# stgl/scarplet

Measured on AMD Instinct MI355X. Metric: Mpixel·template/s (DEM pixels × ages × orientations / s), higher is better.
Workload: dtype f32

## Files before the change

scarplet_amd/csrc/sc_api.hip:

```cpp
#include "sc_internal.h"
#include <stdarg.h>
#include <stdio.h>
#include <string.h>
#include <stdlib.h>
#include <math.h>
#include <algorithm>

int sc_fail(sc_ctx* ctx, int code, const char* fmt, ...) {
    char buf[1024];
    va_list ap;
    va_start(ap, fmt);
    vsnprintf(buf, sizeof(buf), fmt, ap);
    va_end(ap);
    if (ctx) ctx->err = buf;
    return code;
}

int sc_ensure(sc_ctx* ctx, DevBuf& b, size_t bytes) {
    if (bytes <= b.cap && b.p) return SC_OK;
    if (b.p) {
        SC_HIP(ctx, hipFree(b.p));
        b.p = nullptr;
        b.cap = 0;
    }
// ... 27 lines not shown
    size_t s = 0;
    for (DevBuf* b : arr) s += b->cap;
    for (auto& w : c->windows) s += (size_t)w.h * w.wd * 13;
    return s;
}

int sc_lds_attr(sc_ctx* ctx, const void* kernel, size_t bytes) {
    auto it = ctx->lds_attr.find(kernel);
    if (it != ctx->lds_attr.end() && it->second >= bytes) return SC_OK;
    SC_HIP(ctx, hipFuncSetAttribute(kernel, hipFuncAttributeMaxDynamicSharedMemorySize,
                                    (int)bytes));
    ctx->lds_attr[kernel] = bytes;
    return SC_OK;
}

void sc_prof_begin(sc_ctx* ctx, int kernel) {
    ctx->prof_cur = -1;
    ctx->prof_kernel = kernel;
    const long long b = ctx->k_brackets[kernel]++;
    if (!ctx->prof) return;
    uint32_t h = (uint32_t)b * 2654435761u;
    h ^= h >> 15;
    h *= 2246822519u;
    h ^= h >> 13;
    if (ctx->prof > 1 && h % (uint32_t)ctx->prof) return;
    std::pair<hipEvent_t, hipEvent_t> ev;
    if (!ctx->ev_pool.empty()) {
        ev = ctx->ev_pool.back();
        ctx->ev_pool.pop_back();
    } else {
        if (hipEventCreate(&ev.first) != hipSuccess) return;
        if (hipEventCreate(&ev.second) != hipSuccess) return;
    }
    (void)hipEventRecord(ev.first, ctx->stream);
    ctx->prof_cur = kernel;
    ctx->prof_ev0 = ev.first;
    ctx->prof_ev1 = ev.second;
}

void sc_prof_end(sc_ctx* ctx, int n) {
    ctx->k_launches[ctx->prof_kernel] += n;
    if (ctx->prof_cur < 0) return;
    (void)hipEventRecord(ctx->prof_ev1, ctx->stream);
    ctx->pending.push_back({ctx->prof_cur, {ctx->prof_ev0, ctx->prof_ev1}});
    ctx->pending_n.push_back(n);
    ctx->prof_cur = -1;
}

void sc_prof_collect(sc_ctx* ctx) {
    for (size_t i = 0; i < ctx->pending.size(); ++i) {
        auto& p = ctx->pending[i];
        float ms = 0.f;
        if (hipEventElapsedTime(&ms, p.second.first, p.second.second) == hipSuccess) {
            ctx->k_ms[p.first] += ms;
            ctx->k_sampled[p.first] += ctx->pending_n[i];
        }
        ctx->ev_pool.push_back(p.second);
    }
// ... 6 lines not shown
extern "C" int sc_device_count(void) {
    int n = 0;
    if (hipGetDeviceCount(&n) != hipSuccess) return 0;
    return n;
}

extern "C" int sc_create(int device, sc_ctx** out) {
    if (!out) return SC_ERR_INVALID;
    *out = nullptr;
    int n = 0;
    if (hipGetDeviceCount(&n) != hipSuccess || n <= 0) return SC_ERR_HIP;
    if (device < 0 || device >= n) return SC_ERR_INVALID;
    if (hipSetDevice(device) != hipSuccess) return SC_ERR_HIP;
    sc_ctx* c = new sc_ctx();
    c->device = device;
    if (hipStreamCreateWithFlags(&c->stream, hipStreamNonBlocking) != hipSuccess) {
        delete c;
        return SC_ERR_HIP;
    }
    *out = c;
    return SC_OK;
}

extern "C" int sc_set_option(sc_ctx* ctx, const char* name, double value) {
    if (!ctx || !name) return SC_ERR_INVALID;
    if (!strcmp(name, "kappa")) {
        if (!(value >= 0.0)) return sc_fail(ctx, SC_ERR_INVALID, "kappa must be >= 0");
        ctx->kappa = (float)value;
    } else if (!strcmp(name, "variant")) {
        ctx->variant = (int)value;
    } else if (!strcmp(name, "batch")) {
// ... 12 lines not shown
        ctx->batch_templ = (int)value;
    } else if (!strcmp(name, "split_i1")) {
        if (!(value >= 0.0 && value <= 64.0)) return sc_fail(ctx, SC_ERR_INVALID, "split_i1 must be 0 .. 64");
        ctx->split_i1 = (int)value;
    } else if (!strcmp(name, "split_fill")) {
        if (!(value >= 0.0)) return sc_fail(ctx, SC_ERR_INVALID, "split_fill must be >= 0");
        ctx->split_fill = (long long)value;
    } else if (!strcmp(name, "sib")) {
        ctx->sib = (int)value;
    } else if (!strcmp(name, "spectra_mb")) {
        if (!(value >= 0.0)) return sc_fail(ctx, SC_ERR_INVALID, "spectra_mb must be >= 0");
        ctx->spec_mb = value;
        fft_spectra_forget(ctx);
    } else if (!strcmp(name, "fuse_fwd")) {
        ctx->fuse_fwd = value != 0.0;
    } else if (!strcmp(name, "y_gb")) {
        if (!(value >= 0.0)) return sc_fail(ctx, SC_ERR_INVALID, "y_gb must be >= 0");
        ctx->y_gb = value;
    } else if (!strcmp(name, "fit_chunk")) {
        if (!(value >= 0.0 && std::isfinite(value))) return sc_fail(ctx, SC_ERR_INVALID, "fit_chunk must be >= 0 and finite");
        ctx->fit_chunk = value >= 0x1p62 ? (1ll << 62) : (long long)value;
    } else if (!strcmp(name, "channel_terms")) {
        if (!(value == 0.0 || value == 1.0)) return sc_fail(ctx, SC_ERR_INVALID, "channel_terms must be 0 or 1");
        ctx->channel_terms = (int)value;
    } else {
        return sc_fail(ctx, SC_ERR_INVALID, "unknown option '%s'", name);
    }
    return SC_OK;
}

extern "C" int sc_clear_windows(sc_ctx* ctx) {
    if (!ctx) return SC_ERR_INVALID;
    (void)hipStreamSynchronize(ctx->stream);
    for (auto& w : ctx->windows) {
        if (!w.pooled) {
            if (w.w) (void)hipFree(w.w);
            if (w.w64) (void)hipFree(w.w64);
            if (w.m) (void)hipFree(w.m);
        }
        if (w.mask_lim) (void)hipFree(w.mask_lim);
        if (w.mask_err) (void)hipFree(w.mask_err);
    }
    ctx->windows.clear();
    for (void* p : ctx->window_pools) (void)hipFree(p);
    ctx->window_pools.clear();
    return SC_OK;
}

extern "C" void sc_destroy(sc_ctx* c) {
    if (!c) return;
    (void)hipSetDevice(c->device);
    (void)hipStreamSynchronize(c->stream);
    sc_comm_destroy(c);
    sc_prof_collect(c);
    for (auto& e : c->ev_pool) {
        (void)hipEventDestroy(e.first);
        (void)hipEventDestroy(e.second);
    }
    sc_clear_windows(c);
    DevBuf* arr[] = {&c->z, &c->xaxis, &c->yaxis, &c->A, &c->B, &c->C, &c->curv,
                     &c->best_snr, &c->best_amp, &c->best_id, &c->map_amp,
                     &c->map_snr, &c->templ, &c->sums, &c->wl1, &c->norms, &c->norm_part, &c->win_w, &c->win_m,
                     &c->tw_y, &c->tw_x, &c->blk, &c->cblk, &c->uc, &c->uc2, &c->vh, &c->wh, &c->mh,
                     &c->yw, &c->ym, &c->tiles, &c->halo_z, &c->halo_stage, &c->res, &c->sib_buf, &c->dwin, &c->spans, &c->res_stats, &c->digest, &c->split_s, &c->split_a, &c->split_i,
                     &c->near, &c->near_ev, &c->score, &c->score_w, &c->score_abc, &c->st_slot, &c->st_work, &c->st_pairs, &c->st_patch, &c->st_spans, &c->snap, &c->xch, &c->xch_cnt,
                     &c->tr_planes, &c->tr_thin, &c->tr_par, &c->tr_lab, &c->tr_cnt, &c->tr_bsum, &c->tr_tot, &c->tr_sort, &c->tr_hist, &c->tr_rbsum, &c->tr_seg,
                     &c->pf_z, &c->pf_cells, &c->pf_dir, &c->pf_ages, &c->pf_tab, &c->pf_rows, &c->pf_sse, &c->pf_shift, &c->pf_wt, &c->pf_ftab, &c->pf_terms,
                     &c->sg_z, &c->sg_ages, &c->sg_tab, &c->sg_cells, &c->sg_dir, &c->sg_cseg, &c->sg_start, &c->sg_blk, &c->sg_label, &c->sg_prof, &c->sg_int,
                     &c->sg_scal, &c->sg_age, &c->sg_list, &c->sg_part, &c->sg_tot, &c->sg_tsse, &c->sg_cnt, &c->sg_rows, &c->sg_out, &c->sg_sse, &c->sg_shift, &c->sg_ftab, &c->sg_width, &c->sg_fine, &c->sq_wt, &c->sq_state, &c->sq_hist, &c->sq_a,
                     &c->bs_blk, &c->bs_sblk, &c->bs_terms, &c->bs_index, &c->bs_a, &c->bs_hist, &c->bs_rows, &c->cb_rows, &c->cb_mb,
                     &c->st_win, &c->st_wstart, &c->st_spp, &c->st_rows, &c->st_sse, &c->cw_shift,
                     &c->sb_win, &c->sb_wstart, &c->sb_wblk, &c->sb_bhi, &c->sb_rows, &c->sb_hist,
                     &c->sf_work, &c->sf_cells, &c->sf_cube, &c->sf_rows};
    for (DevBuf* b : arr) buf_free(*b);
    for (int k = 0; k < 4; ++k) buf_free(c->cmp[k]);
    for (int k = 0; k < 4; ++k) buf_free(c->cmp_in[k]);
    for (int k = 0; k < 4; ++k) buf_free(c->fill[k]);
    (void)hipStreamDestroy(c->stream);
    delete c;
}

extern "C" const char* sc_last_error(sc_ctx* ctx) {
    return ctx ? ctx->err.c_str() : "null context";
}

extern "C" size_t sc_device_bytes(sc_ctx* ctx) { return ctx ? sc_total_bytes(ctx) : 0; }

static int set_dem_body(sc_ctx* ctx, int ly, int lx, int gy0, int gx0, int ny,
                        int nx, int cy0, int cy1, int cx0, int cx1, double dx,
                        double dy, int wrap, const double* xaxis,
                        const double* yaxis);

// ... 373 lines not shown
    for (int j = 0; j < n; ++j) {
        if (t[j].kind == SC_KIND_WINDOW) ctx->h_wslot[j] = t[j].window;
        ctx->h_mix[3 * (size_t)j] = t[j].cc;
        ctx->h_mix[3 * (size_t)j + 1] = t[j].sc2;
        ctx->h_mix[3 * (size_t)j + 2] = t[j].ss;
        ctx->templ_windows = ctx->templ_windows || t[j].kind == SC_KIND_WINDOW;
    }
}

int sc_load_templates(sc_ctx* ctx, const sc_template* t, int n) {
    sc_plan plan{};
    plan.method = -1;
    int rc = check_templates(ctx, t, n, &plan);
    if (rc) return rc;
    if (ctx->async_in_flight) {
        SC_HIP(ctx, hipStreamSynchronize(ctx->stream));
        ctx->async_in_flight = false;
    }
    std::vector<TemplDev>& h = ctx->h_templ;
    h.assign(n, TemplDev{});
    ctx->h_sums.assign(2 * (size_t)n, 0.0);
    ctx->h_wl1.assign(n, 0.0);
    for (int j = 0; j < n; ++j) templ_from_descriptor(ctx, t[j], h[j], &ctx->h_sums[2 * (size_t)j], &ctx->h_wl1[j]);
    keep_f64_side(ctx, t, n);
    if ((rc = sc_ensure(ctx, ctx->templ, sizeof(TemplDev) * n))) return rc;
    ctx->async_in_flight = true;
    SC_HIP(ctx, hipMemcpyAsync(ctx->templ.p, h.data(), sizeof(TemplDev) * n, hipMemcpyHostToDevice, ctx->stream));
    ctx->last_batch = n;
    return SC_OK;
}

struct CurvState {
    double cur[3] = {0, 0, 0};
    bool have_curv = false;
};
static int chunk_curvature(sc_ctx* ctx, const sc_template* t, const MatchChunk& c, bool fft, const FftGeom& fg, int slot0,
                           CurvState& st) {
    const bool keep = slot0 >= 0;
    bool hit = keep;
    if (keep) {
        ctx->uc_off = (size_t)slot0 * ctx->spec_uc_stride;
        ctx->norms_off = (size_t)slot0 * ctx->spec_norm_stride;
    }
    for (int b = 0; b < c.nb && hit; ++b) {
        const sc_template& sb = t[c.first + b * c.n];
        const double* k = &ctx->spec_key[3 * (size_t)(slot0 + b)];
        hit = k[0] == sb.cc && k[1] == sb.sc2 && k[2] == sb.ss;
    }
    if (hit) {
        st.have_curv = false;
        return SC_OK;
    }
    const sc_template& s0 = t[c.first];
    if (c.nb > 1 || !st.have_curv || s0.cc != st.cur[0] || s0.sc2 != st.cur[1] || s0.ss != st.cur[2]) {
        float coef[SC_MAX_ORIENT][3];
        for (int b = 0; b < c.nb; ++b) {
            const sc_template& sb = t[c.first + b * c.n];
            coef[b][0] = (float)sb.cc; coef[b][1] = (float)sb.sc2; coef[b][2] = (float)sb.ss;
        }
        const bool fused = fft && ctx->variant != 17;
        int rc = SC_OK;
        if (!fused) rc = c.nb > 1 ? launch_curv_alpha_batch(ctx, coef, c.nb) : launch_curv_alpha(ctx, coef[0][0], coef[0][1], coef[0][2]);
        if (rc) return rc;
        if (fft && (rc = fft_forward_curv(ctx, fg, c.nb, fused ? coef : nullptr))) return rc;
        st.cur[0] = s0.cc; st.cur[1] = s0.sc2; st.cur[2] = s0.ss;
        st.have_curv = c.nb == 1;
    }
    for (int b = 0; b < c.nb && keep; ++b) {
        const sc_template& sb = t[c.first + b * c.n];
        double* k = &ctx->spec_key[3 * (size_t)(slot0 + b)];
        k[0] = sb.cc; k[1] = sb.sc2; k[2] = sb.ss;
    }
    return SC_OK;
}

static int match_impl(sc_ctx* ctx, const sc_template* t, int n, const sc_plan* plan,
                      bool to_maps) {
    if (!ctx || !t || !plan || n <= 0) return SC_ERR_INVALID;
    if (!ctx->have_dem) return sc_fail(ctx, SC_ERR_NO_DEM, "no DEM set");
// ... 10 lines not shown
    FftGeom fg{};
    const int group = std::max(1, plan->group);
    if (fft) {
        fg.Ty = plan->Ty; fg.Tx = plan->Tx; fg.Vy = plan->Vy; fg.Vx = plan->Vx;
        fg.nty = plan->nty; fg.ntx = plan->ntx; fg.circ_y = plan->circ_y;
        fg.circ_x = plan->circ_x; fg.Py = plan->Py; fg.Qx = plan->Qx;
        fg.ntiles = fg.nty * fg.ntx;
    }
    if (to_maps) {
        size_t nc = (size_t)(g.cy1 - g.cy0) * (g.cx1 - g.cx0);
        if ((rc = sc_ensure(ctx, ctx->map_amp, sizeof(float) * nc))) return rc;
        if ((rc = sc_ensure(ctx, ctx->map_snr, sizeof(float) * nc))) return rc;
    }

    if (ctx->async_in_flight) {
        SC_HIP(ctx, hipStreamSynchronize(ctx->stream));
        ctx->async_in_flight = false;
    }
    std::vector<TemplDev>& h = ctx->h_templ;
    std::vector<double>&sums = ctx->h_sums, &wl1 = ctx->h_wl1;
    std::vector<unsigned char>& masked = ctx->h_masked;
    h.assign(n, TemplDev{});
    sums.assign(2 * (size_t)n, 0.0);
    wl1.assign(n, 0.0);
    masked.assign(n, 0);
    for (int j = 0; j < n; ++j) {
        templ_from_descriptor(ctx, t[j], h[j], &sums[2 * (size_t)j], &wl1[j]);
        masked[j] = h[j].mask_lim != nullptr || h[j].mask_err != nullptr;
    }
    MatchPlanIn in{};
    in.t = t; in.n = n; in.masked = masked.data();
// ... 21 lines not shown
        if ((rc = sc_ensure(ctx, ctx->spans, sizeof(int4) * std::max<size_t>(mp.max_spans, 1)))) return rc;
    }
    ctx->async_in_flight = true;
    SC_HIP(ctx, hipMemcpyAsync(ctx->templ.p, h.data(), sizeof(TemplDev) * n,
                               hipMemcpyHostToDevice, ctx->stream));
    SC_HIP(ctx, hipMemcpyAsync(ctx->sums.p, sums.data(), sizeof(double) * 2 * n,
                               hipMemcpyHostToDevice, ctx->stream));
    SC_HIP(ctx, hipMemcpyAsync(ctx->wl1.p, wl1.data(), sizeof(double) * n,
                               hipMemcpyHostToDevice, ctx->stream));
    ctx->last_batch = n;
    keep_f64_side(ctx, t, n);

    CurvState curv;
    for (const MatchChunk& c : mp.chunks) {
        const int n_all = c.nb * c.n;
        if ((rc = chunk_curvature(ctx, t, c, fft, fg, keep ? mp.slot_of[c.run0] : -1, curv))) return rc;
        for (int j = c.first; j < c.first + n_all; ++j) {
            if (t[j].kind != SC_KIND_WINDOW) continue;
            const WindowSlot& w = ctx->windows[t[j].window];
            size_t cells = (size_t)w.h * w.wd;
            SC_HIP(ctx, hipMemcpyAsync((float*)ctx->win_w.p + h[j].win_off, w.w,
                                       cells * sizeof(float), hipMemcpyDeviceToDevice, ctx->stream));
            SC_HIP(ctx, hipMemcpyAsync((uint8_t*)ctx->win_m.p + h[j].win_off, w.m, cells,
                                       hipMemcpyDeviceToDevice, ctx->stream));
        }
        if ((rc = launch_windows(ctx, c.first, n_all, c.wh, c.ww))) return rc;
        if (!fft) {
            if ((rc = launch_direct(ctx, c.first, c.n, to_maps, c.nb, c.wh, c.ww, c.long_runs))) return rc;
        } else {
            if ((rc = fft_forward_templates(ctx, fg, c.first, n_all, c.parity))) return rc;
            if ((rc = fft_inverse_fold(ctx, fg, c.first, c.n, group, to_maps, c.full, c.parity, c.nb))) return rc;
        }
    }
    return SC_OK;
}

extern "C" int sc_match_async(sc_ctx* ctx, const sc_template* t, int n, const sc_plan* plan) {
    int rc = match_impl(ctx, t, n, plan, false);
    if (ctx) ctx->async_in_flight = true;
    return rc;
}

extern "C" int sc_sync(sc_ctx* ctx) {
    if (!ctx) return SC_ERR_INVALID;
    SC_HIP(ctx, hipSetDevice(ctx->device));
    SC_HIP(ctx, hipStreamSynchronize(ctx->stream));
    ctx->async_in_flight = false;
    sc_prof_collect(ctx);
    return SC_OK;
}

extern "C" int sc_match(sc_ctx* ctx, const sc_template* t, int n, const sc_plan* plan) {
    int rc = match_impl(ctx, t, n, plan, false);
    if (rc) return rc;
    return sc_sync(ctx);
}

extern "C" int sc_match_template(sc_ctx* ctx, const sc_template* t, const sc_plan* plan,
                                 float* amp, float* snr) {
    if (!amp || !snr) return SC_ERR_INVALID;
    int rc = match_impl(ctx, t, 1, plan, true);
// ... 199 lines not shown
```

scarplet_amd/csrc/sc_fft.hip:

```cpp
#include "sc_internal.h"
#include <math.h>
#include <type_traits>
#include <string.h>

struct TileDev {
    int i0, j0, vy, vx, gi0, gj0;
};

__host__ __device__ constexpr int fft_threads(int T) {
    return (T / 4) >= 512 ? 512 : ((T / 4) < 64 ? 64 : (T / 4));
}
__host__ __device__ constexpr int fft_waves(int T) { return T >= 4096 ? 2 : 4; }
__host__ __device__ constexpr int fft_line(int T) { return T + T / 16 + 8; }
__host__ __device__ constexpr size_t fft_lds_bytes(int T) {
    return (size_t)4 * fft_line(T) * sizeof(float2);
}
__device__ __forceinline__ int ph(int i) { return i + (i >> 4); }

__device__ __forceinline__ void lds_barrier() {
    asm volatile("s_waitcnt lgkmcnt(0)" ::: "memory");
    __builtin_amdgcn_s_barrier();
    asm volatile("" ::: "memory");
}
__device__ __forceinline__ void store_stream(float2* dst, float2 a, float2 b) {
// ... 2240 lines not shown
    in.Ty = fg.Ty; in.Tx = fg.Tx; in.ntiles = fg.ntiles; in.parity = parity;
    in.near = ctx->near_w > 0.f; in.kept = ctx->spec_slots > 0;
    in.nb = in.n = in.group = 1;
    in.variant = ctx->variant; in.sib = ctx->sib; in.i1_pairs = ctx->i1_pairs; in.split_i1 = ctx->split_i1;
    in.split_fill = ctx->split_fill; in.fuse_fwd = ctx->fuse_fwd; in.batch_off = ctx->batch_off;
    in.batch_templ = ctx->batch_templ; in.batch_fill = ctx->batch_fill;
    return in;
}

static bool fft_fuse_curv(const sc_ctx* ctx, const FftGeom& fg, int slots) {
    FftRouteIn in = fft_route_in(ctx, fg, 1);
    in.kept = slots > 0;
    return fft_route(in).fused;
}

void fft_spectra_forget(sc_ctx* ctx) {
    std::fill(ctx->spec_key.begin(), ctx->spec_key.end(), NAN);
}

int fft_prepare(sc_ctx* ctx, const FftGeom& fg, int n_templ_chunk, int group, int nb, int n_slots) {
    if (!fft_size_supported(fg.Ty) || !fft_size_supported(fg.Tx))
        return sc_fail(ctx, SC_ERR_UNSUPPORTED, FFT_REFUSE_SIZE, fg.Ty, fg.Tx);
    int rc;
    if ((rc = upload_twiddles(ctx, ctx->tw_y, ctx->tw_Ty, fg.Ty, 1 - ctx->g.oy))) return rc;
    if ((rc = upload_twiddles(ctx, ctx->tw_x, ctx->tw_Tx, fg.Tx, 1 - ctx->g.ox))) return rc;
    const Geom& g = ctx->g;
    int np = npairs_of(fg);
    std::vector<TileDev> h(2 * np);
    for (int k = 0; k < 2 * np; ++k) {
        TileDev t{0, 0, 0, 0, 0, 0};
// ... 99 lines not shown
}

template <typename K>
static int set_lds(sc_ctx* ctx, K kernel, size_t bytes) {
    return sc_lds_attr(ctx, (const void*)kernel, bytes);
}

template <int... Ts, typename F>
static int fft_for_size(sc_ctx* ctx, int size, const char* fmt, F f) {
    int rc = SC_OK;
    const bool matched = ((size == Ts && ((rc = f(std::integral_constant<int, Ts>{})), true)) || ...);
    return matched ? rc : sc_fail(ctx, SC_ERR_UNSUPPORTED, fmt, size);
}
#define FFT_SIZES 64, 128, 256, 512, 1024, 2048, 4096

static int launch_fwd_cols(sc_ctx* ctx, const FftGeom& fg, const float2* in, int nplanes,
                           float2* out0, float2* out1, int split2,
                           const TemplDev* templ = nullptr) {
    size_t lds = fft_lds_bytes(fg.Ty);
    dim3 grid(fg.Tx / 4, nplanes);
    sc_prof_begin(ctx, SC_K_FWD_COLS);
    int rc = fft_for_size<FFT_SIZES>(ctx, fg.Ty, "tile size %d", [&](auto t) {
        constexpr int T = decltype(t)::value;
        if (int rc = set_lds(ctx, k_fwd_cols<T>, lds)) return rc;
        hipLaunchKernelGGL(k_fwd_cols<T>, grid, dim3(fft_threads(T)), lds, ctx->stream, in, fg.Tx,
                           (const float2*)ctx->tw_y.p, out0, out1, split2, templ);
        return SC_OK;
    });
    if (rc) return rc;
    sc_prof_end(ctx);
    SC_HIP(ctx, hipGetLastError());
    return SC_OK;
}

int fft_forward_curv(sc_ctx* ctx, const FftGeom& fg, int nb, const float (*coef)[3]) {
    int np = npairs_of(fg);
    size_t lds = fft_lds_bytes(fg.Tx);
    dim3 grid(fg.Ty / 4 / FWD_ROWS_RBW, np * nb);
    const bool fuse = fft_fuse_curv(ctx, fg, ctx->spec_slots);
    float2* rows_out = (float2*)(fuse ? ctx->cblk.p : ctx->blk.p);
// ... 12 lines not shown
            hipLaunchKernelGGL(kernel, grid, dim3(fft_threads(T)), lds, ctx->stream, (const float*)plane,
                               (const float*)ctx->B.p, (const float*)ctx->C.p, mixc, ctx->g,
                               (const TileDev*)ctx->tiles.p, fg.Ty, (const float2*)ctx->tw_x.p, rows_out,
                               (double*)ctx->norm_part.p, np, (size_t)ctx->g.ly * ctx->g.lx);
            return SC_OK;
        };
        return coef ? launch(k_fwd_rows_curv<T, true>, ctx->A.p) : launch(k_fwd_rows_curv<T, false>, ctx->curv.p);
    });
    if (rc) return rc;
    hipLaunchKernelGGL(k_tile_norms, dim3(np * nb), dim3(64), 0, ctx->stream,
                       (const double*)ctx->norm_part.p, fg.Ty / 4, (double*)ctx->norms.p + ctx->norms_off);
    sc_prof_end(ctx);
    SC_HIP(ctx, hipGetLastError());
    ctx->curv_rows = fuse ? 2 * np * nb : 0;
    if (fuse) return SC_OK;
    return launch_fwd_cols(ctx, fg, rows_out, 2 * np * nb, (float2*)ctx->uc.p + ctx->uc_off, (float2*)ctx->uc2.p + ctx->uc_off, 1);
}

int fft_forward_templates(sc_ctx* ctx, const FftGeom& fg, int first, int n, int parity) {
    size_t lds = fft_lds_bytes(fg.Tx);
    dim3 grid(fg.Ty / 4, n);
    sc_prof_begin(ctx, SC_K_FWD_ROWS);
    int rc = fft_for_size<FFT_SIZES>(ctx, fg.Tx, "tile size %d", [&](auto t) {
        constexpr int T = decltype(t)::value;
        if (int rc = set_lds(ctx, k_fwd_rows_templ<T>, lds)) return rc;
        hipLaunchKernelGGL(k_fwd_rows_templ<T>, grid, dim3(fft_threads(T)), lds, ctx->stream,
                           (const TemplDev*)ctx->templ.p, first, (const float*)ctx->win_w.p,
                           (const uint8_t*)ctx->win_m.p, (const double*)ctx->sums.p, fg.Ty,
                           (const float2*)ctx->tw_x.p, (float2*)ctx->blk.p);
        return SC_OK;
    });
    if (rc) return rc;
    sc_prof_end(ctx);
    SC_HIP(ctx, hipGetLastError());
    const FftTemplFwd how = fft_route(fft_route_in(ctx, fg, parity)).templ;
    if (how == FFT_TEMPL_COLS_SYM) {
        size_t ldsc = fft_lds_bytes(fg.Ty);
        dim3 gridc(fg.Tx / 8 + 1, n);
        sc_prof_begin(ctx, SC_K_FWD_COLS);
        rc = fft_for_size<64, 128, 256, 512, 1024, 2048>(ctx, fg.Ty, "symmetric template transform: column length %d", [&](auto t) {
            constexpr int T = decltype(t)::value;
            if (int rc = set_lds(ctx, k_fwd_cols_tsym<T>, ldsc)) return rc;
            hipLaunchKernelGGL(k_fwd_cols_tsym<T>, gridc, dim3(fft_threads(T)), ldsc, ctx->stream,
                               (const float2*)ctx->blk.p, fg.Tx, (const float2*)ctx->tw_y.p,
                               (const TemplDev*)ctx->templ.p + first, (const float2*)ctx->tw_x.p + fg.Tx,
                               parity, (float*)ctx->wh.p, (float*)ctx->mh.p);
            return SC_OK;
        });
        if (rc) return rc;
        sc_prof_end(ctx);
        SC_HIP(ctx, hipGetLastError());
        return SC_OK;
    }
    rc = launch_fwd_cols(ctx, fg, (const float2*)ctx->blk.p, n, (float2*)ctx->vh.p, nullptr, 0,
                         (const TemplDev*)ctx->templ.p + first);
    if (rc) return rc;
    size_t cells = half_plane(fg.Ty, fg.Tx);
    dim3 grid_s((unsigned)((cells / 2 + 255) / 256), n);
    sc_prof_begin(ctx, SC_K_FWD_COLS);
    if (how == FFT_TEMPL_SPLIT_SYM)
        hipLaunchKernelGGL(k_split_templ_sym, grid_s, dim3(256), 0, ctx->stream,
                           (const float2*)ctx->vh.p, fg.Ty, fg.Tx, (const float2*)ctx->tw_y.p + fg.Ty,
                           (const float2*)ctx->tw_x.p + fg.Tx,
                           parity, (float*)ctx->wh.p, (float*)ctx->mh.p);
    else
        hipLaunchKernelGGL(k_split_templ, grid_s, dim3(256), 0, ctx->stream, (const float2*)ctx->vh.p,
                           fg.Ty, fg.Tx, (float2*)ctx->wh.p, (float2*)ctx->mh.p);
    sc_prof_end(ctx);
    SC_HIP(ctx, hipGetLastError());
    return SC_OK;
}

struct ColLaunch {
    int Ty, Tx;
    bool pt;
    int jobs;
    int ng;
    int split_i1;
    const float2 *uc, *uc2;
    const void *wh, *mh;
    int pair, vfirst, G, rp_lo, rp_hi;
// ... 192 lines not shown
    int np = npairs_of(fg);
    int rp_lo = 0, rp_hi = fg.Ty / 2 - 1;
    if (!fg.circ_y) {
        rp_lo = fg.Py / 2;
        rp_hi = std::min(fg.Ty - 1, fg.Py + fg.Vy - 1) / 2;
    }
    const int rp_n = rp_hi - rp_lo + 1;
    const int pb = std::max(1, ctx->fft_pb);
    const size_t yblock = (size_t)fg.Ty * fg.Tx * group;
    const bool fwd = ctx->curv_rows > 0 && r.fwd;
    if (ctx->curv_rows > 0 && !fwd) {
        const size_t half = (size_t)fg.Ty * fg.Tx * sizeof(float2) * (ctx->curv_rows / 2);
        int rc;
        if ((rc = sc_ensure(ctx, ctx->uc, half))) return rc;
        if ((rc = sc_ensure(ctx, ctx->uc2, half))) return rc;
        if ((rc = launch_fwd_cols(ctx, fg, (const float2*)ctx->cblk.p, ctx->curv_rows, (float2*)ctx->uc.p + ctx->uc_off,
                                  (float2*)ctx->uc2.p + ctx->uc_off, 1)))
            return rc;
        ctx->curv_rows = 0;
    }
    auto chunk = [&](int pair0, int pc, bool pt) -> int {
        const FftChunkRoute& c = pt ? r.ptc : r.main;
        const bool xp = fft_route_xp(c.col), fast = c.row != FFT_ROW_GENERIC;
        for (int g0 = 0; g0 < n; g0 += group) {
            int G = std::min(group, n - g0);
            const int ng = fft_route_transforms(G, pt);
            const FftColPairs cp = fft_route_col_pairs(c, fg.Ty, fg.Tx, nb, pc);
            sc_prof_begin(ctx, SC_K_INV_COLS);
            int n_i1 = 0;
            for (int pl0 = 0; pl0 < pc; pl0 += cp.pairs) {
                const int pcc = std::min(cp.pairs, pc - pl0);
// ... 91 lines not shown
```

scarplet_amd/csrc/sc_fft_route.h:

```cpp
#pragma once
#include "../../include/scarplet_hip.h"

#define SC_MAX_GROUP 64
#define SC_MAX_BATCH 256
#define SC_MAX_ORIENT 64

enum FftColKernel {
    FFT_COL_GENERIC,
    FFT_COL_SYM,
    FFT_COL_SYMX,
    FFT_COL_SYMX_XP,
    FFT_COL_W8,
    FFT_COL_W4,
    FFT_COL_H2,
    FFT_COL_H2_XP
};
enum FftRowKernel {
    FFT_ROW_GENERIC,
    FFT_ROW_FAST,
    FFT_ROW_NEAR,
    FFT_ROW_SPLIT
};
enum FftTemplFwd {
    FFT_TEMPL_SPLIT,
// ... 85 lines not shown
                                                          : FFT_COL_GENERIC;
        c.jil = c.col == FFT_COL_W8 && in.nb == 1 && v != 1 && in.i1_pairs > 1 ? in.i1_pairs : 1;
        const bool split = fast && !(in.near && xp) && !in.to_maps && !in.full_masks && Tx <= 1024 && v != 15 &&
                           !(in.sib & 1);
        c.row = !fast ? FFT_ROW_GENERIC : split ? FFT_ROW_SPLIT : r.near ? FFT_ROW_NEAR : FFT_ROW_FAST;
        c.split_min_g = in.near ? 4 : 1;
        c.split_max = v == 20 ? 1 : 4;
        c.split_waves = in.split_fill > 0 ? in.split_fill : 4300;
        return c;
    };
    r.main = chunk(false);
    r.ptc = chunk(true);
    return r;
}

inline int fft_route_batch(const FftRouteIn& in) {
    if (in.batch_off || in.n < 1 || in.n > in.group || !fft_route_fast(in)) return 1;
    const int np = (in.ntiles + 1) / 2;
    const int cap = in.batch_templ > 0 ? in.batch_templ : SC_MAX_BATCH;
    const int capg = cap < SC_MAX_GROUP ? cap : SC_MAX_GROUP;
    const int by_table = (SC_MAX_GROUP / in.n >= 3 || cap <= SC_MAX_GROUP) ? capg / in.n : cap / in.n;
    const int wgs = np * (in.Tx / 8);
    const int by_fill = (in.batch_fill > 0 ? in.batch_fill : 4096) / (wgs > 1 ? wgs : 1);
    int nb = by_table < by_fill ? by_table : by_fill;
    if (nb > SC_MAX_ORIENT) nb = SC_MAX_ORIENT;
    return nb > 1 ? nb : 1;
}

inline int fft_route_parts(int split_i1, long long workgroups, long long capacity, int transforms) {
    if (!split_i1 || workgroups <= 0) return 1;
// ... 57 lines not shown
```

scarplet_amd/csrc/sc_internal.h:

```cpp
#pragma once
#include <hip/hip_runtime.h>
#include <stdint.h>
#include <string>
#include <vector>
#include <map>
#include <limits.h>
#include "../../include/scarplet_hip.h"

#define SC_EPS 2.220446049250313e-16
#define SC_EVENT_WORDS 4

#define SC_EXP_UNDERFLOW 745.1332191019412

struct TemplDev {
    int32_t kind, flags;
    double cos_a, sin_a, c, d, p0, p1;
    int32_t ilo, ihi, jlo, jhi;
    int32_t pmin, pmax, qmin, qmax;
    uint32_t id;
    int32_t wh, ww;
    long long win_off;
    long long dwin_off;
    int32_t dpitch, span_off;
    const uint8_t* mask_lim;
// ... 25 lines not shown
    double* w64 = nullptr;
    uint8_t* m = nullptr;
    int h = 0, wd = 0;
    uint8_t* mask_lim = nullptr;
    uint8_t* mask_err = nullptr;
    bool pooled = false;
};

#include "sc_fft_route.h"
#include "sc_direct_route.h"
#include "sc_match_plan.h"

struct sc_ctx {
    int device = 0;
    hipStream_t stream = nullptr;
    std::string err;
    bool have_dem = false;
    Geom g{};
    double dx = 1, dy = 1;
    DevBuf z, xaxis, yaxis, A, B, C, curv;
    bool z_borrowed = false;
    const double* z_dev = nullptr;
    unsigned long long dem_hash[2] = {0, 0};
    long long dem_nan = 0;
    double dem_sig[16] = {0};
    bool dem_unchanged = false;
    DevBuf digest;
    DevBuf best_snr, best_amp, best_id;
    DevBuf map_amp, map_snr;
    DevBuf cmp[4], cmp_in[4];
// ... 47 lines not shown
    long long split_fill = 0;
    int variant = 0;
    int batch_off = 0;
    int i1_pairs = 2;
    int batch_fill = 0;
    double y_gb = 0.0;
    int sib = 0;
    long long fit_chunk = 0;
    int channel_terms = 1;
    DevBuf split_s, split_a, split_i;
    DevBuf sib_buf;
    uint32_t sib_epoch = 0;
    int prof = 0;
    int prof_cur = -1;
    hipEvent_t prof_ev0 = nullptr, prof_ev1 = nullptr;
    long long k_launches[SC_K_COUNT] = {0};
    long long k_brackets[SC_K_COUNT] = {0};
    int prof_kernel = 0;
    std::vector<int> pending_n;
    long long k_sampled[SC_K_COUNT] = {0};
    double k_ms[SC_K_COUNT] = {0};
    std::vector<std::pair<int, std::pair<hipEvent_t, hipEvent_t>>> pending;
    std::vector<std::pair<hipEvent_t, hipEvent_t>> ev_pool;
    std::map<const void*, size_t> lds_attr;
    void* comm = nullptr;
    int rank = 0, nranks = 1;
    DevBuf halo_z, halo_stage;
    DevBuf res;
    DevBuf fill[4];
    DevBuf tr_planes, tr_thin, tr_par, tr_lab, tr_cnt, tr_bsum, tr_tot, tr_sort, tr_hist, tr_rbsum, tr_seg;
// ... 19 lines not shown
};

int sc_fail(sc_ctx* ctx, int code, const char* fmt, ...);
int sc_ensure(sc_ctx* ctx, DevBuf& b, size_t bytes);
size_t sc_total_bytes(sc_ctx* ctx);
int sc_lds_attr(sc_ctx* ctx, const void* kernel, size_t bytes);

#define SC_HIP(ctx, call)                                                     \
    do {                                                                      \
        hipError_t e__ = (call);                                              \
        if (e__ != hipSuccess)                                                \
            return sc_fail(ctx, SC_ERR_HIP, "%s: %s (%s:%d)", #call,          \
                           hipGetErrorString(e__), __FILE__, __LINE__);       \
    } while (0)

void sc_prof_begin(sc_ctx* ctx, int kernel);
void sc_prof_end(sc_ctx* ctx, int n = 1);
void sc_prof_collect(sc_ctx* ctx);
#define SC_RECORD_BYTES 12
int sc_launch_result(sc_ctx* ctx, const float* amp, const float* snr, const uint32_t* id, const double* tab_par,
                     const double* tab_ang, int n_ids, size_t n, double* planes);
int sc_load_templates(sc_ctx* ctx, const sc_template* t, int n);
int sc_near_buffers(sc_ctx* ctx, unsigned long long** ev_count, uint32_t** ev, unsigned long long* ev_cap);
int sc_window_runs(sc_ctx* ctx, int n, const unsigned long long* woff, const double* wbuf, double* sums, unsigned* soff, int* maxlen);
int sc_apply_patches(sc_ctx* ctx, const double* tab_par, const double* tab_ang, int n_ids, size_t nc, double* planes);
int sc_result_planes(sc_ctx* ctx, const double* param_of_id, const double* angle_of_id, int n_ids,
                     double** planes_out, size_t* nc_out);

int launch_curv_planes(sc_ctx* ctx);
int launch_dem_digest(sc_ctx* ctx, unsigned long long* out_dev);
int launch_curv_alpha(sc_ctx* ctx, float cc, float sc2, float ss, int plane = 0);
int launch_curv_f64(sc_ctx* ctx, double c2, double sn, double cs, double s2, double* out_dev);
int launch_curv_alpha_batch(sc_ctx* ctx, const float (*coef)[3], int nb);
int score_prepare_f64(sc_ctx* ctx, int n_templ, const unsigned long long** woff_out, const double** wbuf_out, const double** planes_out,
                      const double** mix_out);
int launch_score_f64(sc_ctx* ctx, const int* cells_dev, const int* tsel_dev, int m, int n_templ, double* amp_dev, double* snr_dev);
int launch_windows(sc_ctx* ctx, int first, int n, int wh_max, int ww_max);
int launch_direct(sc_ctx* ctx, int first, int n, bool to_maps, int nb, int wh_max, int ww_max, bool long_runs);
bool direct_window_fits(int ww);
int launch_fill_nodata(sc_ctx* ctx, double* zdev, double* tmp, int* up, int* dn, int ny, int nx,
                       double maxd, int smoothing, unsigned long long* remaining_dev);
int launch_compare_fold(sc_ctx* ctx, double age, double angle, bool planes);

int fft_prepare(sc_ctx* ctx, const FftGeom& fg, int n_templ_chunk, int group, int nb, int n_slots);
void fft_spectra_forget(sc_ctx* ctx);
FftRouteIn fft_route_in(const sc_ctx* ctx, const FftGeom& fg, int parity);
int fft_forward_curv(sc_ctx* ctx, const FftGeom& fg, int nb, const float (*coef)[3] = nullptr);
int fft_forward_templates(sc_ctx* ctx, const FftGeom& fg, int first, int n, int parity);
int fft_inverse_fold(sc_ctx* ctx, const FftGeom& fg, int first, int n,
                     int group, bool to_maps, bool full_masks, int parity, int nb);
bool fft_size_supported(int T);

#ifdef __HIPCC__
__device__ __forceinline__ int wrap_index(int g, int n) {
    g %= n;
    return g < 0 ? g + n : g;
}

__device__ __forceinline__ float load_curv(const float* __restrict__ curv,
                                           const Geom& g, int gi, int gj) {
    int li, lj;
    if (g.wrap) {
        li = wrap_index(gi, g.ny);
// ... 96 lines not shown
```

scarplet_amd/csrc/sc_kernels.hip:

```cpp
#include "sc_internal.h"
#include <algorithm>
#include <string.h>

template <typename OUT>
__global__ void __launch_bounds__(256)
k_curv_planes(const double* __restrict__ z, Geom g, double dx, double dy,
              OUT* __restrict__ A, OUT* __restrict__ B,
              OUT* __restrict__ C) {
    int j = blockIdx.x * blockDim.x + threadIdx.x;
    int i = blockIdx.y;
    if (j >= g.lx) return;
    int gi = wrap_index(g.gy0 + i, g.ny);
    int gj = wrap_index(g.gx0 + j, g.nx);
    int im = max(i - 1, 0), ip = min(i + 1, g.ly - 1);
    int jm = max(j - 1, 0), jp = min(j + 1, g.lx - 1);
    const double* r0 = z + (size_t)im * g.lx;
    const double* r1 = z + (size_t)i * g.lx;
    const double* r2 = z + (size_t)ip * g.lx;
    double z11 = r1[j];
    double a = 0.0, b = 0.0, c = 0.0;
    if (gj >= 1 && gj <= g.nx - 2)
        a = __ddiv_rn(__dsub_rn(__dsub_rn(r1[jp], z11), __dsub_rn(z11, r1[jm])),
                      __dmul_rn(dx, dx));
    if (gi >= 1 && gj >= 1) {
// ... 1080 lines not shown
int launch_curv_alpha(sc_ctx* ctx, float cc, float sc2, float ss, int plane) {
    size_t n = (size_t)ctx->g.ly * ctx->g.lx;
    size_t blocks = (n / 4 + 255) / 256;
    if (blocks > 8192) blocks = 8192;
    if (blocks < 1) blocks = 1;
    sc_prof_begin(ctx, SC_K_CURV);
    hipLaunchKernelGGL(k_curv_alpha, dim3((unsigned)blocks), dim3(256), 0,
                       ctx->stream, (const float*)ctx->A.p,
                       (const float*)ctx->B.p, (const float*)ctx->C.p, cc, sc2,
                       ss, (float*)ctx->curv.p + (size_t)plane * n, n);
    sc_prof_end(ctx);
    SC_HIP(ctx, hipGetLastError());
    return SC_OK;
}

int launch_windows(sc_ctx* ctx, int first, int n, int wh_max, int ww_max) {
    if (n <= 0 || wh_max <= 0 || ww_max <= 0) return SC_OK;
    dim3 grid((ww_max + 63) / 64, (wh_max + SC_WIN_ROWS - 1) / SC_WIN_ROWS, n);
    sc_prof_begin(ctx, SC_K_WINDOWS);
    hipLaunchKernelGGL(k_windows, grid, dim3(64), 0, ctx->stream,
                       (const TemplDev*)ctx->templ.p, first,
                       (const double*)ctx->xaxis.p, (const double*)ctx->yaxis.p,
                       ctx->g.ny, ctx->g.nx, (float*)ctx->win_w.p,
                       (uint8_t*)ctx->win_m.p, (double*)ctx->sums.p,
                       (double*)ctx->wl1.p);
    sc_prof_end(ctx);
    SC_HIP(ctx, hipGetLastError());
    return SC_OK;
}

bool direct_window_fits(int ww) {
    const long long p2 = 256 + ((ww + 3) & ~3);
    return p2 * 16 <= DR2_LDS_FLOATS && (long long)(((DR_TX + ww - 1) | 1)) * DR_TY <= DR_LDS_FLOATS;
}

// ... 74 lines not shown
```

Baseline: 194,800.

## Overlap template forward FFT with curvature FFT on a second stream

Adds a second HIP stream with fork/join events so that, for fused FFT routes without window copies or map output, template window construction and forward template FFTs run concurrently with the curvature forward transform. The goal is to fill idle compute units while the two independent forward stages proceed, then join before the inverse fold. Adds event and synchronisation overhead, and stream-wide syncs are replaced with a drain of both streams. This carries some risk of contention or races on shared buffers.

After: 194,700 (median of 2 runs). No clear change (-0.1%).

```diff
diff --git a/scarplet_amd/csrc/sc_api.hip b/scarplet_amd/csrc/sc_api.hip
--- a/scarplet_amd/csrc/sc_api.hip
+++ b/scarplet_amd/csrc/sc_api.hip
@@ -65,9 +65,10 @@
     return SC_OK;
 }
 
-void sc_prof_begin(sc_ctx* ctx, int kernel) {
+void sc_prof_begin(sc_ctx* ctx, int kernel, hipStream_t stream) {
     ctx->prof_cur = -1;
     ctx->prof_kernel = kernel;
+    ctx->prof_stream = stream ? stream : ctx->stream;
     const long long b = ctx->k_brackets[kernel]++;
     if (!ctx->prof) return;
     uint32_t h = (uint32_t)b * 2654435761u;
@@ -83,7 +84,7 @@
         if (hipEventCreate(&ev.first) != hipSuccess) return;
         if (hipEventCreate(&ev.second) != hipSuccess) return;
     }
-    (void)hipEventRecord(ev.first, ctx->stream);
+    (void)hipEventRecord(ev.first, ctx->prof_stream);
     ctx->prof_cur = kernel;
     ctx->prof_ev0 = ev.first;
     ctx->prof_ev1 = ev.second;
@@ -92,7 +93,7 @@
 void sc_prof_end(sc_ctx* ctx, int n) {
     ctx->k_launches[ctx->prof_kernel] += n;
     if (ctx->prof_cur < 0) return;
-    (void)hipEventRecord(ctx->prof_ev1, ctx->stream);
+    (void)hipEventRecord(ctx->prof_ev1, ctx->prof_stream);
     ctx->pending.push_back({ctx->prof_cur, {ctx->prof_ev0, ctx->prof_ev1}});
     ctx->pending_n.push_back(n);
     ctx->prof_cur = -1;
@@ -129,7 +130,13 @@
     if (hipSetDevice(device) != hipSuccess) return SC_ERR_HIP;
     sc_ctx* c = new sc_ctx();
     c->device = device;
-    if (hipStreamCreateWithFlags(&c->stream, hipStreamNonBlocking) != hipSuccess) {
+    if (hipStreamCreateWithFlags(&c->stream, hipStreamNonBlocking) != hipSuccess ||
+        hipStreamCreateWithFlags(&c->stream2, hipStreamNonBlocking) != hipSuccess ||
+        hipEventCreateWithFlags(&c->ev_fork, hipEventDisableTiming) != hipSuccess ||
+        hipEventCreateWithFlags(&c->ev_join, hipEventDisableTiming) != hipSuccess) {
+        if (c->ev_fork) (void)hipEventDestroy(c->ev_fork);
+        if (c->stream2) (void)hipStreamDestroy(c->stream2);
+        if (c->stream) (void)hipStreamDestroy(c->stream);
         delete c;
         return SC_ERR_HIP;
     }
@@ -172,6 +179,8 @@
         fft_spectra_forget(ctx);
     } else if (!strcmp(name, "fuse_fwd")) {
         ctx->fuse_fwd = value != 0.0;
+    } else if (!strcmp(name, "fwd_overlap")) {
+        ctx->fwd_overlap = value != 0.0;
     } else if (!strcmp(name, "y_gb")) {
         if (!(value >= 0.0)) return sc_fail(ctx, SC_ERR_INVALID, "y_gb must be >= 0");
         ctx->y_gb = value;
@@ -187,9 +196,15 @@
     return SC_OK;
 }
 
+int sc_drain(sc_ctx* ctx) {
+    SC_HIP(ctx, hipStreamSynchronize(ctx->stream2));
+    SC_HIP(ctx, hipStreamSynchronize(ctx->stream));
+    return SC_OK;
+}
+
 extern "C" int sc_clear_windows(sc_ctx* ctx) {
     if (!ctx) return SC_ERR_INVALID;
-    (void)hipStreamSynchronize(ctx->stream);
+    (void)sc_drain(ctx);
     for (auto& w : ctx->windows) {
         if (!w.pooled) {
             if (w.w) (void)hipFree(w.w);
@@ -208,7 +223,7 @@
 extern "C" void sc_destroy(sc_ctx* c) {
     if (!c) return;
     (void)hipSetDevice(c->device);
-    (void)hipStreamSynchronize(c->stream);
+    (void)sc_drain(c);
     sc_comm_destroy(c);
     sc_prof_collect(c);
     for (auto& e : c->ev_pool) {
@@ -234,6 +249,9 @@
     for (int k = 0; k < 4; ++k) buf_free(c->cmp[k]);
     for (int k = 0; k < 4; ++k) buf_free(c->cmp_in[k]);
     for (int k = 0; k < 4; ++k) buf_free(c->fill[k]);
+    (void)hipEventDestroy(c->ev_fork);
+    (void)hipEventDestroy(c->ev_join);
+    (void)hipStreamDestroy(c->stream2);
     (void)hipStreamDestroy(c->stream);
     delete c;
 }
@@ -637,7 +655,7 @@
     int rc = check_templates(ctx, t, n, &plan);
     if (rc) return rc;
     if (ctx->async_in_flight) {
-        SC_HIP(ctx, hipStreamSynchronize(ctx->stream));
+        if (int rcd = sc_drain(ctx)) return rcd;
         ctx->async_in_flight = false;
     }
     std::vector<TemplDev>& h = ctx->h_templ;
@@ -656,11 +674,13 @@
 struct CurvState {
     double cur[3] = {0, 0, 0};
     bool have_curv = false;
+    bool launched = false;
 };
 static int chunk_curvature(sc_ctx* ctx, const sc_template* t, const MatchChunk& c, bool fft, const FftGeom& fg, int slot0,
                            CurvState& st) {
     const bool keep = slot0 >= 0;
     bool hit = keep;
+    st.launched = false;
     if (keep) {
         ctx->uc_off = (size_t)slot0 * ctx->spec_uc_stride;
         ctx->norms_off = (size_t)slot0 * ctx->spec_norm_stride;
@@ -686,6 +706,7 @@
         if (!fused) rc = c.nb > 1 ? launch_curv_alpha_batch(ctx, coef, c.nb) : launch_curv_alpha(ctx, coef[0][0], coef[0][1], coef[0][2]);
         if (rc) return rc;
         if (fft && (rc = fft_forward_curv(ctx, fg, c.nb, fused ? coef : nullptr))) return rc;
+        st.launched = true;
         st.cur[0] = s0.cc; st.cur[1] = s0.sc2; st.cur[2] = s0.ss;
         st.have_curv = c.nb == 1;
     }
@@ -726,7 +747,7 @@
     }
 
     if (ctx->async_in_flight) {
-        SC_HIP(ctx, hipStreamSynchronize(ctx->stream));
+        if (int rcd = sc_drain(ctx)) return rcd;
         ctx->async_in_flight = false;
     }
     std::vector<TemplDev>& h = ctx->h_templ;
@@ -778,7 +799,17 @@
     CurvState curv;
     for (const MatchChunk& c : mp.chunks) {
         const int n_all = c.nb * c.n;
+        bool window_copies = false;
+        for (int j = c.first; j < c.first + n_all; ++j) window_copies |= t[j].kind == SC_KIND_WINDOW;
+        const bool may_fork = fft && fft_forward_overlap(ctx, fg, to_maps, window_copies, true);
+        if (may_fork) SC_HIP(ctx, hipEventRecord(ctx->ev_fork, ctx->stream));
         if ((rc = chunk_curvature(ctx, t, c, fft, fg, keep ? mp.slot_of[c.run0] : -1, curv))) return rc;
+        const bool fork = may_fork && fft_forward_overlap(ctx, fg, to_maps, window_copies, curv.launched);
+        hipStream_t ts = ctx->stream;
+        if (fork) {
+            ts = ctx->stream2;
+            SC_HIP(ctx, hipStreamWaitEvent(ts, ctx->ev_fork, 0));
+        }
         for (int j = c.first; j < c.first + n_all; ++j) {
             if (t[j].kind != SC_KIND_WINDOW) continue;
             const WindowSlot& w = ctx->windows[t[j].window];
@@ -788,11 +819,15 @@
             SC_HIP(ctx, hipMemcpyAsync((uint8_t*)ctx->win_m.p + h[j].win_off, w.m, cells,
                                        hipMemcpyDeviceToDevice, ctx->stream));
         }
-        if ((rc = launch_windows(ctx, c.first, n_all, c.wh, c.ww))) return rc;
+        if ((rc = launch_windows(ctx, ts, c.first, n_all, c.wh, c.ww))) return rc;
         if (!fft) {
             if ((rc = launch_direct(ctx, c.first, c.n, to_maps, c.nb, c.wh, c.ww, c.long_runs))) return rc;
         } else {
-            if ((rc = fft_forward_templates(ctx, fg, c.first, n_all, c.parity))) return rc;
+            if ((rc = fft_forward_templates(ctx, ts, fg, c.first, n_all, c.parity))) return rc;
+            if (fork) {
+                SC_HIP(ctx, hipEventRecord(ctx->ev_join, ts));
+                SC_HIP(ctx, hipStreamWaitEvent(ctx->stream, ctx->ev_join, 0));
+            }
             if ((rc = fft_inverse_fold(ctx, fg, c.first, c.n, group, to_maps, c.full, c.parity, c.nb))) return rc;
         }
     }
@@ -808,7 +843,7 @@
 extern "C" int sc_sync(sc_ctx* ctx) {
     if (!ctx) return SC_ERR_INVALID;
     SC_HIP(ctx, hipSetDevice(ctx->device));
-    SC_HIP(ctx, hipStreamSynchronize(ctx->stream));
+    if (int rc = sc_drain(ctx)) return rc;
     ctx->async_in_flight = false;
     sc_prof_collect(ctx);
     return SC_OK;
diff --git a/scarplet_amd/csrc/sc_fft.hip b/scarplet_amd/csrc/sc_fft.hip
--- a/scarplet_amd/csrc/sc_fft.hip
+++ b/scarplet_amd/csrc/sc_fft.hip
@@ -2278,6 +2278,11 @@
     return fft_route(in).fused;
 }
 
+bool fft_forward_overlap(const sc_ctx* ctx, const FftGeom& fg, bool to_maps, bool window_copies, bool curv_launched) {
+    FftRouteIn in = fft_route_in(ctx, fg, 1);
+    return fft_route_fwd_overlap(fft_route(in), ctx->fwd_overlap != 0, to_maps, window_copies, curv_launched);
+}
+
 void fft_spectra_forget(sc_ctx* ctx) {
     std::fill(ctx->spec_key.begin(), ctx->spec_key.end(), NAN);
 }
@@ -2407,16 +2412,16 @@
 }
 #define FFT_SIZES 64, 128, 256, 512, 1024, 2048, 4096
 
-static int launch_fwd_cols(sc_ctx* ctx, const FftGeom& fg, const float2* in, int nplanes,
+static int launch_fwd_cols(sc_ctx* ctx, hipStream_t stream, const FftGeom& fg, const float2* in, int nplanes,
                            float2* out0, float2* out1, int split2,
                            const TemplDev* templ = nullptr) {
     size_t lds = fft_lds_bytes(fg.Ty);
     dim3 grid(fg.Tx / 4, nplanes);
-    sc_prof_begin(ctx, SC_K_FWD_COLS);
+    sc_prof_begin(ctx, SC_K_FWD_COLS, stream);
     int rc = fft_for_size<FFT_SIZES>(ctx, fg.Ty, "tile size %d", [&](auto t) {
         constexpr int T = decltype(t)::value;
         if (int rc = set_lds(ctx, k_fwd_cols<T>, lds)) return rc;
-        hipLaunchKernelGGL(k_fwd_cols<T>, grid, dim3(fft_threads(T)), lds, ctx->stream, in, fg.Tx,
+        hipLaunchKernelGGL(k_fwd_cols<T>, grid, dim3(fft_threads(T)), lds, stream, in, fg.Tx,
                            (const float2*)ctx->tw_y.p, out0, out1, split2, templ);
         return SC_OK;
     });
@@ -2459,17 +2464,17 @@
     SC_HIP(ctx, hipGetLastError());
     ctx->curv_rows = fuse ? 2 * np * nb : 0;
     if (fuse) return SC_OK;
-    return launch_fwd_cols(ctx, fg, rows_out, 2 * np * nb, (float2*)ctx->uc.p + ctx->uc_off, (float2*)ctx->uc2.p + ctx->uc_off, 1);
-}
-
-int fft_forward_templates(sc_ctx* ctx, const FftGeom& fg, int first, int n, int parity) {
+    return launch_fwd_cols(ctx, ctx->stream, fg, rows_out, 2 * np * nb, (float2*)ctx->uc.p + ctx->uc_off, (float2*)ctx->uc2.p + ctx->uc_off, 1);
+}
+
+int fft_forward_templates(sc_ctx* ctx, hipStream_t stream, const FftGeom& fg, int first, int n, int parity) {
     size_t lds = fft_lds_bytes(fg.Tx);
     dim3 grid(fg.Ty / 4, n);
-    sc_prof_begin(ctx, SC_K_FWD_ROWS);
+    sc_prof_begin(ctx, SC_K_FWD_ROWS, stream);
     int rc = fft_for_size<FFT_SIZES>(ctx, fg.Tx, "tile size %d", [&](auto t) {
         constexpr int T = decltype(t)::value;
         if (int rc = set_lds(ctx, k_fwd_rows_templ<T>, lds)) return rc;
-        hipLaunchKernelGGL(k_fwd_rows_templ<T>, grid, dim3(fft_threads(T)), lds, ctx->stream,
+        hipLaunchKernelGGL(k_fwd_rows_templ<T>, grid, dim3(fft_threads(T)), lds, stream,
                            (const TemplDev*)ctx->templ.p, first, (const float*)ctx->win_w.p,
                            (const uint8_t*)ctx->win_m.p, (const double*)ctx->sums.p, fg.Ty,
                            (const float2*)ctx->tw_x.p, (float2*)ctx->blk.p);
@@ -2482,11 +2487,11 @@
     if (how == FFT_TEMPL_COLS_SYM) {
         size_t ldsc = fft_lds_bytes(fg.Ty);
         dim3 gridc(fg.Tx / 8 + 1, n);
-        sc_prof_begin(ctx, SC_K_FWD_COLS);
+        sc_prof_begin(ctx, SC_K_FWD_COLS, stream);
         rc = fft_for_size<64, 128, 256, 512, 1024, 2048>(ctx, fg.Ty, "symmetric template transform: column length %d", [&](auto t) {
             constexpr int T = decltype(t)::value;
             if (int rc = set_lds(ctx, k_fwd_cols_tsym<T>, ldsc)) return rc;
-            hipLaunchKernelGGL(k_fwd_cols_tsym<T>, gridc, dim3(fft_threads(T)), ldsc, ctx->stream,
+            hipLaunchKernelGGL(k_fwd_cols_tsym<T>, gridc, dim3(fft_threads(T)), ldsc, stream,
                                (const float2*)ctx->blk.p, fg.Tx, (const float2*)ctx->tw_y.p,
                                (const TemplDev*)ctx->templ.p + first, (const float2*)ctx->tw_x.p + fg.Tx,
                                parity, (float*)ctx->wh.p, (float*)ctx->mh.p);
@@ -2497,19 +2502,19 @@
         SC_HIP(ctx, hipGetLastError());
         return SC_OK;
     }
-    rc = launch_fwd_cols(ctx, fg, (const float2*)ctx->blk.p, n, (float2*)ctx->vh.p, nullptr, 0,
+    rc = launch_fwd_cols(ctx, stream, fg, (const float2*)ctx->blk.p, n, (float2*)ctx->vh.p, nullptr, 0,
                          (const TemplDev*)ctx->templ.p + first);
     if (rc) return rc;
     size_t cells = half_plane(fg.Ty, fg.Tx);
     dim3 grid_s((unsigned)((cells / 2 + 255) / 256), n);
-    sc_prof_begin(ctx, SC_K_FWD_COLS);
+    sc_prof_begin(ctx, SC_K_FWD_COLS, stream);
     if (how == FFT_TEMPL_SPLIT_SYM)
-        hipLaunchKernelGGL(k_split_templ_sym, grid_s, dim3(256), 0, ctx->stream,
+        hipLaunchKernelGGL(k_split_templ_sym, grid_s, dim3(256), 0, stream,
                            (const float2*)ctx->vh.p, fg.Ty, fg.Tx, (const float2*)ctx->tw_y.p + fg.Ty,
                            (const float2*)ctx->tw_x.p + fg.Tx,
                            parity, (float*)ctx->wh.p, (float*)ctx->mh.p);
     else
-        hipLaunchKernelGGL(k_split_templ, grid_s, dim3(256), 0, ctx->stream, (const float2*)ctx->vh.p,
+        hipLaunchKernelGGL(k_split_templ, grid_s, dim3(256), 0, stream, (const float2*)ctx->vh.p,
                            fg.Ty, fg.Tx, (float2*)ctx->wh.p, (float2*)ctx->mh.p);
     sc_prof_end(ctx);
     SC_HIP(ctx, hipGetLastError());
@@ -2732,7 +2737,7 @@
         int rc;
         if ((rc = sc_ensure(ctx, ctx->uc, half))) return rc;
         if ((rc = sc_ensure(ctx, ctx->uc2, half))) return rc;
-        if ((rc = launch_fwd_cols(ctx, fg, (const float2*)ctx->cblk.p, ctx->curv_rows, (float2*)ctx->uc.p + ctx->uc_off,
+        if ((rc = launch_fwd_cols(ctx, ctx->stream, fg, (const float2*)ctx->cblk.p, ctx->curv_rows, (float2*)ctx->uc.p + ctx->uc_off,
                                   (float2*)ctx->uc2.p + ctx->uc_off, 1)))
             return rc;
         ctx->curv_rows = 0;
diff --git a/scarplet_amd/csrc/sc_fft_route.h b/scarplet_amd/csrc/sc_fft_route.h
--- a/scarplet_amd/csrc/sc_fft_route.h
+++ b/scarplet_amd/csrc/sc_fft_route.h
@@ -123,6 +123,10 @@
     return r;
 }
 
+inline bool fft_route_fwd_overlap(const FftRoute& r, bool option, bool to_maps, bool window_copies, bool curv_launched) {
+    return option && !r.err && r.fused && !to_maps && !window_copies && curv_launched;
+}
+
 inline int fft_route_batch(const FftRouteIn& in) {
     if (in.batch_off || in.n < 1 || in.n > in.group || !fft_route_fast(in)) return 1;
     const int np = (in.ntiles + 1) / 2;
diff --git a/scarplet_amd/csrc/sc_internal.h b/scarplet_amd/csrc/sc_internal.h
--- a/scarplet_amd/csrc/sc_internal.h
+++ b/scarplet_amd/csrc/sc_internal.h
@@ -63,6 +63,9 @@
 struct sc_ctx {
     int device = 0;
     hipStream_t stream = nullptr;
+    hipStream_t stream2 = nullptr;
+    hipEvent_t ev_fork = nullptr, ev_join = nullptr;
+    int fwd_overlap = 1;
     std::string err;
     bool have_dem = false;
     Geom g{};
@@ -140,6 +143,7 @@
     int prof = 0;
     int prof_cur = -1;
     hipEvent_t prof_ev0 = nullptr, prof_ev1 = nullptr;
+    hipStream_t prof_stream = nullptr;
     long long k_launches[SC_K_COUNT] = {0};
     long long k_brackets[SC_K_COUNT] = {0};
     int prof_kernel = 0;
@@ -189,7 +193,9 @@
                            hipGetErrorString(e__), __FILE__, __LINE__);       \
     } while (0)
 
-void sc_prof_begin(sc_ctx* ctx, int kernel);
+int sc_drain(sc_ctx* ctx);
+
+void sc_prof_begin(sc_ctx* ctx, int kernel, hipStream_t stream = nullptr);
 void sc_prof_end(sc_ctx* ctx, int n = 1);
 void sc_prof_collect(sc_ctx* ctx);
 #define SC_RECORD_BYTES 12
@@ -210,7 +216,7 @@
 int score_prepare_f64(sc_ctx* ctx, int n_templ, const unsigned long long** woff_out, const double** wbuf_out, const double** planes_out,
                       const double** mix_out);
 int launch_score_f64(sc_ctx* ctx, const int* cells_dev, const int* tsel_dev, int m, int n_templ, double* amp_dev, double* snr_dev);
-int launch_windows(sc_ctx* ctx, int first, int n, int wh_max, int ww_max);
+int launch_windows(sc_ctx* ctx, hipStream_t stream, int first, int n, int wh_max, int ww_max);
 int launch_direct(sc_ctx* ctx, int first, int n, bool to_maps, int nb, int wh_max, int ww_max, bool long_runs);
 bool direct_window_fits(int ww);
 int launch_fill_nodata(sc_ctx* ctx, double* zdev, double* tmp, int* up, int* dn, int ny, int nx,
@@ -221,7 +227,8 @@
 void fft_spectra_forget(sc_ctx* ctx);
 FftRouteIn fft_route_in(const sc_ctx* ctx, const FftGeom& fg, int parity);
 int fft_forward_curv(sc_ctx* ctx, const FftGeom& fg, int nb, const float (*coef)[3] = nullptr);
-int fft_forward_templates(sc_ctx* ctx, const FftGeom& fg, int first, int n, int parity);
+int fft_forward_templates(sc_ctx* ctx, hipStream_t stream, const FftGeom& fg, int first, int n, int parity);
+bool fft_forward_overlap(const sc_ctx* ctx, const FftGeom& fg, bool to_maps, bool window_copies, bool curv_launched);
 int fft_inverse_fold(sc_ctx* ctx, const FftGeom& fg, int first, int n,
                      int group, bool to_maps, bool full_masks, int parity, int nb);
 bool fft_size_supported(int T);
diff --git a/scarplet_amd/csrc/sc_kernels.hip b/scarplet_amd/csrc/sc_kernels.hip
--- a/scarplet_amd/csrc/sc_kernels.hip
+++ b/scarplet_amd/csrc/sc_kernels.hip
@@ -1118,11 +1118,11 @@
     return SC_OK;
 }
 
-int launch_windows(sc_ctx* ctx, int first, int n, int wh_max, int ww_max) {
+int launch_windows(sc_ctx* ctx, hipStream_t stream, int first, int n, int wh_max, int ww_max) {
     if (n <= 0 || wh_max <= 0 || ww_max <= 0) return SC_OK;
     dim3 grid((ww_max + 63) / 64, (wh_max + SC_WIN_ROWS - 1) / SC_WIN_ROWS, n);
-    sc_prof_begin(ctx, SC_K_WINDOWS);
-    hipLaunchKernelGGL(k_windows, grid, dim3(64), 0, ctx->stream,
+    sc_prof_begin(ctx, SC_K_WINDOWS, stream);
+    hipLaunchKernelGGL(k_windows, grid, dim3(64), 0, stream,
                        (const TemplDev*)ctx->templ.p, first,
                        (const double*)ctx->xaxis.p, (const double*)ctx->yaxis.p,
                        ctx->g.ny, ctx->g.nx, (float*)ctx->win_w.p,
```
